# liuzuxin/FSRL

Hardware: NVIDIA H100
Metric: env-steps/sec (collect+update) SafetyCarCircle-v0 PPO-Lag (higher is better)
Workload: dtype f32

## Files before the change

fsrl_b200/csrc/mlp.cuh:

```cuda
#pragma once
#include "arena.cuh"
#include <cuda_pipeline.h>

namespace fsrl {

constexpr int MLP_TPB = 256;
constexpr int MLP_KC = 16;
constexpr int MLP_NST = 4;
constexpr int MLP_MAX_OUT = 16;
constexpr int MLP_MAX_IN = 64;

template <int H>
struct MlpTile {
    static_assert(H == 64 || H == 128 || H == 256 || H == 512, "hidden width must be 64/128/256/512");
    static constexpr int R = (4096 / H) < 16 ? 16 : (4096 / H);
    static constexpr int MT = R / 16;
    static constexpr int WN = H / 8;
    static constexpr int NT = WN / 8;
    static constexpr int LDA = H + 4;
    static constexpr int LDW = H + 8;
    static constexpr int PARTS = MLP_TPB / R;
    static constexpr int NST = (H >= 512) ? 2 : MLP_NST;
    __host__ __device__ static constexpr int in_pad(int in) { return ((in + 7) & ~7) + 4; }
    __host__ __device__ static constexpr int stage_floats() { return NST * MLP_KC * LDW; }
    __host__ __device__ static constexpr size_t smem_floats(int in, int out) {
        return (size_t)R * in_pad(in) + 2 * (size_t)R * LDA + stage_floats() + (size_t)H * out;
    }
    __host__ __device__ static constexpr size_t smem_bytes(int in, int out = MLP_MAX_OUT) {
        return sizeof(float) * smem_floats(in, out);
    }
};

__device__ __forceinline__ uint32_t round_tf32(float x) { return (__float_as_uint(x) + 0x1000u) & 0xffffe000u; }
__device__ __forceinline__ void split_tf32(float x, uint32_t& hi, uint32_t& lo) {
    hi = round_tf32(x);
    lo = round_tf32(x - __uint_as_float(hi));
}

__device__ __forceinline__ void mma_tf32(float (&c)[4], const uint32_t (&a)[4], const uint32_t (&b)[2]) {
    asm(
        "mma.sync.aligned.m16n8k8.row.col.f32.tf32.tf32.f32 {%0,%1,%2,%3}, {%4,%5,%6,%7}, {%8,%9}, {%0,%1,%2,%3};"
        : "+f"(c[0]), "+f"(c[1]), "+f"(c[2]), "+f"(c[3])
        : "r"(a[0]), "r"(a[1]), "r"(a[2]), "r"(a[3]), "r"(b[0]), "r"(b[1]));
}

template <int H>
__device__ __forceinline__ void stage_load(const float* mat, int K, float* wst, int chunk, int buf) {
    using TT = MlpTile<H>;
    float* dst = wst + (size_t)buf * MLP_KC * TT::LDW;
    constexpr int SEG = H / 4;
    for (int i = threadIdx.x; i < MLP_KC * SEG; i += MLP_TPB) {
        const int rr = i / SEG, sg = i % SEG;
        const int k = chunk * MLP_KC + rr;
        float* d = dst + (size_t)rr * TT::LDW + 4 * sg;
        if (k < K) __pipeline_memcpy_async(d, mat + (size_t)k * H + 4 * sg, 16);
        else *reinterpret_cast<float4*>(d) = make_float4(0.f, 0.f, 0.f, 0.f);
    }
    __pipeline_commit();
}

template <int H>
__device__ __forceinline__ void tc_gemm(float (&c)[MlpTile<H>::MT][MlpTile<H>::NT][4], const float* A,
                                        int lda, int K, const float* W, float* wst,
                                        bool stage0_in_flight) {
    using TT = MlpTile<H>;
    const int lane = threadIdx.x & 31, warp = threadIdx.x >> 5;
    const int g = lane >> 2, t = lane & 3;
    const int n0 = warp * TT::WN;
    const int Kp = (K + 7) & ~7;
    const int nch = (Kp + MLP_KC - 1) / MLP_KC;
    for (int p = stage0_in_flight ? 1 : 0; p < TT::NST - 1; ++p) {
        if (p < nch) stage_load<H>(W, K, wst, p, p);
        else __pipeline_commit();
    }
    for (int ch = 0; ch < nch; ++ch) {
        if (ch + TT::NST - 1 < nch) stage_load<H>(W, K, wst, ch + TT::NST - 1, (ch + TT::NST - 1) % TT::NST);
        else __pipeline_commit();
        __pipeline_wait_prior(TT::NST - 1);
        __syncthreads();
        const float* w = wst + (size_t)(ch % TT::NST) * MLP_KC * TT::LDW;
        const int kleft = Kp - ch * MLP_KC;
#pragma unroll
        for (int ks = 0; ks < MLP_KC; ks += 8) {
            if (ks < kleft) {
                const int k0 = ch * MLP_KC + ks;
                uint32_t bh[TT::NT][2], bl[TT::NT][2];
#pragma unroll
                for (int nt = 0; nt < TT::NT; ++nt) {
                    split_tf32(w[(size_t)(ks + t) * TT::LDW + n0 + 8 * nt + g], bh[nt][0], bl[nt][0]);
                    split_tf32(w[(size_t)(ks + t + 4) * TT::LDW + n0 + 8 * nt + g], bh[nt][1], bl[nt][1]);
                }
#pragma unroll
                for (int mt = 0; mt < TT::MT; ++mt) {
                    uint32_t ah[4], al[4];
                    const float* a = A + (size_t)(16 * mt + g) * lda + k0 + t;
                    split_tf32(a[0], ah[0], al[0]);
                    split_tf32(a[(size_t)8 * lda], ah[1], al[1]);
                    split_tf32(a[4], ah[2], al[2]);
                    split_tf32(a[(size_t)8 * lda + 4], ah[3], al[3]);
#pragma unroll
                    for (int nt = 0; nt < TT::NT; ++nt) mma_tf32(c[mt][nt], al, bh[nt]);
#pragma unroll
                    for (int nt = 0; nt < TT::NT; ++nt) mma_tf32(c[mt][nt], ah, bl[nt]);
#pragma unroll
                    for (int nt = 0; nt < TT::NT; ++nt) mma_tf32(c[mt][nt], ah, bh[nt]);
                }
            }
        }
        __syncthreads();
    }
}

template <int H, class F>
__device__ __forceinline__ void tc_foreach(float (&c)[MlpTile<H>::MT][MlpTile<H>::NT][4], F f) {
    using TT = MlpTile<H>;
    const int lane = threadIdx.x & 31, warp = threadIdx.x >> 5;
    const int g = lane >> 2, t = lane & 3;
#pragma unroll
    for (int mt = 0; mt < TT::MT; ++mt)
#pragma unroll
        for (int nt = 0; nt < TT::NT; ++nt) {
            const int col = warp * TT::WN + 8 * nt + 2 * t;
            f(16 * mt + g, col, c[mt][nt][0], c[mt][nt][1]);
            f(16 * mt + g + 8, col, c[mt][nt][2], c[mt][nt][3]);
        }
}

template <int H>
__device__ __forceinline__ void tc_init_bias(float (&c)[MlpTile<H>::MT][MlpTile<H>::NT][4], const float* bias) {
    using TT = MlpTile<H>;
    const int lane = threadIdx.x & 31, warp = threadIdx.x >> 5;
    const int t = lane & 3;
#pragma unroll
    for (int nt = 0; nt < TT::NT; ++nt) {
        const int col = warp * TT::WN + 8 * nt + 2 * t;
        const float b0 = bias ? __ldg(bias + col) : 0.f, b1 = bias ? __ldg(bias + col + 1) : 0.f;
#pragma unroll
        for (int mt = 0; mt < TT::MT; ++mt) { c[mt][nt][0] = b0; c[mt][nt][1] = b1; c[mt][nt][2] = b0; c[mt][nt][3] = b1; }
    }
}


constexpr int SLAB_NS = 64;
constexpr int SLAB_LDB = SLAB_NS + 8;
constexpr int SLAB_LDR = SLAB_NS + 4;

template <int H>
__host__ __device__ constexpr size_t slab_b_floats() { return (size_t)H * SLAB_LDB; }
template <int H>
__host__ __device__ constexpr size_t slab_red_floats() { return (size_t)8 * MlpTile<H>::R * SLAB_LDR; }
template <int H>
__host__ __device__ constexpr size_t slab_buf_floats() {
    return slab_b_floats<H>() > slab_red_floats<H>() ? slab_b_floats<H>() : slab_red_floats<H>();
}

template <int H>
__device__ __forceinline__ void slab_load(const float* W, int gld, int c0, float* bs) {
    constexpr int SEG = SLAB_NS / 4;
    for (int i = threadIdx.x; i < H * SEG; i += MLP_TPB) {
        const int k = i / SEG, sg = i % SEG;
        __pipeline_memcpy_async(bs + (size_t)k * SLAB_LDB + 4 * sg, W + (size_t)k * gld + c0 + 4 * sg, 16);
    }
    __pipeline_commit();
}

template <int H, class F>
__device__ __forceinline__ void slab_gemm(const float* A, int lda, const float* bs, float* red, F epi) {
    using TT = MlpTile<H>;
    constexpr int NTS = SLAB_NS / 8;
    constexpr int KW = H / 8;
    const int lane = threadIdx.x & 31, warp = threadIdx.x >> 5;
    const int g = lane >> 2, t = lane & 3;
    float c[TT::MT][NTS][4];
#pragma unroll
    for (int mt = 0; mt < TT::MT; ++mt)
#pragma unroll
        for (int nt = 0; nt < NTS; ++nt) { c[mt][nt][0] = c[mt][nt][1] = c[mt][nt][2] = c[mt][nt][3] = 0.f; }
#pragma unroll
    for (int ks = 0; ks < KW; ks += 8) {
        const int k0 = warp * KW + ks;
        uint32_t bh[NTS][2], bl[NTS][2];
#pragma unroll
        for (int nt = 0; nt < NTS; ++nt) {
            split_tf32(bs[(size_t)(k0 + t) * SLAB_LDB + 8 * nt + g], bh[nt][0], bl[nt][0]);
            split_tf32(bs[(size_t)(k0 + t + 4) * SLAB_LDB + 8 * nt + g], bh[nt][1], bl[nt][1]);
        }
#pragma unroll
        for (int mt = 0; mt < TT::MT; ++mt) {
            uint32_t ah[4], al[4];
            const float* a = A + (size_t)(16 * mt + g) * lda + k0 + t;
            split_tf32(a[0], ah[0], al[0]);
            split_tf32(a[(size_t)8 * lda], ah[1], al[1]);
            split_tf32(a[4], ah[2], al[2]);
            split_tf32(a[(size_t)8 * lda + 4], ah[3], al[3]);
#pragma unroll
            for (int nt = 0; nt < NTS; ++nt) mma_tf32(c[mt][nt], al, bh[nt]);
#pragma unroll
            for (int nt = 0; nt < NTS; ++nt) mma_tf32(c[mt][nt], ah, bl[nt]);
#pragma unroll
            for (int nt = 0; nt < NTS; ++nt) mma_tf32(c[mt][nt], ah, bh[nt]);
        }
    }
    __pipeline_wait_prior(0);
    __syncthreads();
    float* mine = red + (size_t)warp * TT::R * SLAB_LDR;
#pragma unroll
    for (int mt = 0; mt < TT::MT; ++mt)
#pragma unroll
        for (int nt = 0; nt < NTS; ++nt) {
            *reinterpret_cast<float2*>(mine + (size_t)(16 * mt + g) * SLAB_LDR + 8 * nt + 2 * t) = make_float2(c[mt][nt][0], c[mt][nt][1]);
            *reinterpret_cast<float2*>(mine + (size_t)(16 * mt + g + 8) * SLAB_LDR + 8 * nt + 2 * t) = make_float2(c[mt][nt][2], c[mt][nt][3]);
        }
    __syncthreads();
    for (int e = threadIdx.x; e < TT::R * (SLAB_NS / 4); e += MLP_TPB) {
        const int row = e / (SLAB_NS / 4), c4 = (e % (SLAB_NS / 4)) * 4;
        float4 s = make_float4(0.f, 0.f, 0.f, 0.f);
#pragma unroll
        for (int w = 0; w < 8; ++w) {
            const float4 v = *reinterpret_cast<const float4*>(red + ((size_t)w * TT::R + row) * SLAB_LDR + c4);
            s.x += v.x; s.y += v.y; s.z += v.z; s.w += v.w;
        }
        epi(row, c4, s);
    }
}

template <int H>
__device__ __forceinline__ void tc_gemm_direct(float (&c)[MlpTile<H>::MT][MlpTile<H>::NT][4], const float* A,
                                               int lda, int K, const float* W) {
    using TT = MlpTile<H>;
    const int lane = threadIdx.x & 31, warp = threadIdx.x >> 5;
    const int g = lane >> 2, t = lane & 3;
    const int n0 = warp * TT::WN;
    const int Kp = (K + 7) & ~7;
    for (int k0 = 0; k0 < Kp; k0 += 8) {
        uint32_t bh[TT::NT][2], bl[TT::NT][2];
#pragma unroll
        for (int nt = 0; nt < TT::NT; ++nt) {
            const float w0 = (k0 + t < K) ? __ldg(W + (size_t)(k0 + t) * H + n0 + 8 * nt + g) : 0.f;
            const float w1 = (k0 + t + 4 < K) ? __ldg(W + (size_t)(k0 + t + 4) * H + n0 + 8 * nt + g) : 0.f;
            split_tf32(w0, bh[nt][0], bl[nt][0]);
            split_tf32(w1, bh[nt][1], bl[nt][1]);
        }
#pragma unroll
        for (int mt = 0; mt < TT::MT; ++mt) {
            uint32_t ah[4], al[4];
            const float* a = A + (size_t)(16 * mt + g) * lda + k0 + t;
            split_tf32(a[0], ah[0], al[0]);
            split_tf32(a[(size_t)8 * lda], ah[1], al[1]);
            split_tf32(a[4], ah[2], al[2]);
            split_tf32(a[(size_t)8 * lda + 4], ah[3], al[3]);
#pragma unroll
            for (int nt = 0; nt < TT::NT; ++nt) mma_tf32(c[mt][nt], al, bh[nt]);
#pragma unroll
            for (int nt = 0; nt < TT::NT; ++nt) mma_tf32(c[mt][nt], ah, bl[nt]);
#pragma unroll
            for (int nt = 0; nt < TT::NT; ++nt) mma_tf32(c[mt][nt], ah, bh[nt]);
        }
    }
}

template <int H>
struct MlpSmem {
    float *x, *h1, *h2, *wst, *w3s;
    __device__ MlpSmem(float* base, int in, int out) {
        using TT = MlpTile<H>;
        x = base;
        h1 = x + (size_t)TT::R * TT::in_pad(in);
        h2 = h1 + (size_t)TT::R * TT::LDA;
        wst = h2 + (size_t)TT::R * TT::LDA;
        w3s = wst + TT::stage_floats();
        (void)out;
    }
    __device__ float* end(int out) const { return w3s + (size_t)H * out; }
};

template <int H>
__device__ __forceinline__ void mlp_hidden_forward(const Mlp3& m, const MlpSmem<H>& s) {
    using TT = MlpTile<H>;
    const int inp = TT::in_pad(m.in);
    for (int i = threadIdx.x; i < H * m.out; i += MLP_TPB) s.w3s[i] = __ldg(m.w3t + i);
    float c[TT::MT][TT::NT][4];
    tc_init_bias<H>(c, m.b1);
    tc_gemm<H>(c, s.x, inp, m.in, m.w1t, s.wst, false);
    stage_load<H>(m.w2t, H, s.wst, 0, 0);
    tc_foreach<H>(c, [&](int row, int col, float v0, float v1) {
        *reinterpret_cast<float2*>(s.h1 + (size_t)row * TT::LDA + col) = make_float2(fmaxf(v0, 0.f), fmaxf(v1, 0.f));
    });
    tc_init_bias<H>(c, m.b2);
    tc_gemm<H>(c, s.h1, TT::LDA, H, m.w2t, s.wst, true);
    tc_foreach<H>(c, [&](int row, int col, float v0, float v1) {
        *reinterpret_cast<float2*>(s.h2 + (size_t)row * TT::LDA + col) = make_float2(fmaxf(v0, 0.f), fmaxf(v1, 0.f));
    });
    __syncthreads();
}

template <int H>
__device__ __forceinline__ void mlp_head_forward(const Mlp3& m, const MlpSmem<H>& s, float* out) {
    using TT = MlpTile<H>;
    const int tid = threadIdx.x;
    const int r = tid / TT::PARTS, part = tid % TT::PARTS;
    const int no = m.out;
#pragma unroll
    for (int j = 0; j < MLP_MAX_OUT; ++j) out[j] = 0.f;
    for (int k = part; k < H; k += TT::PARTS) {
        const float x = s.h2[(size_t)r * TT::LDA + k];
        const float* w = s.w3s + (size_t)k * no;
#pragma unroll
        for (int j = 0; j < MLP_MAX_OUT; ++j)
            if (j < no) out[j] = fmaf(x, w[j], out[j]);
    }
#pragma unroll
    for (int j = 0; j < MLP_MAX_OUT; ++j) {
        if (j < no) {
            float v = out[j];
#pragma unroll
            for (int o = TT::PARTS / 2; o > 0; o >>= 1) v += __shfl_down_sync(0xffffffffu, v, o, TT::PARTS);
            out[j] = v + __ldg(m.b3 + j);
        }
    }
}

template <int H, class RowPtr>
__device__ __forceinline__ void mlp_stage_rows(const MlpSmem<H>& s, int in, RowPtr row_ptr) {
    using TT = MlpTile<H>;
    const int inp = TT::in_pad(in);
    for (int i = threadIdx.x; i < TT::R * inp; i += MLP_TPB) {
        const int r = i / inp, k = i % inp;
        const float* p = row_ptr(r);
        s.x[i] = (p != nullptr && k < in) ? p[k] : 0.f;
    }
}

}
```

fsrl_b200/csrc/mlpfwd.cu:

```cuda
#include "mlp.cuh"
#include "fsrl_b200.h"

namespace fsrl {

template <int H>
__global__ void __launch_bounds__(MLP_TPB)
mlp_forward_kernel(const Mlp3 m, const float* __restrict__ x, const int* __restrict__ idx,
                   long long n_rows, float* __restrict__ y) {
    using TT = MlpTile<H>;
    extern __shared__ __align__(16) float smem[];
    const int tid = threadIdx.x;
    const MlpSmem<H> sm(smem, m.in, m.out);
    const long long r0 = (long long)blockIdx.x * TT::R;
    mlp_stage_rows<H>(sm, m.in, [&](int r) -> const float* {
        const long long row = r0 + r;
        if (row >= n_rows) return nullptr;
        const long long src = idx ? (long long)idx[row] : row;
        return x + src * m.in;
    });
    __syncthreads();
    mlp_hidden_forward<H>(m, sm);
    float out[MLP_MAX_OUT];
    mlp_head_forward<H>(m, sm, out);
    const int r = tid / TT::PARTS, part = tid % TT::PARTS;
    const long long row = r0 + r;
    if (part == 0 && row < n_rows) {
#pragma unroll
        for (int j = 0; j < MLP_MAX_OUT; ++j)
            if (j < m.out) y[row * m.out + j] = out[j];
    }
}

}

using namespace fsrl;

extern "C" int fsrl_mlp_forward(const fsrl_mlp3_t* net, const float* x, const int* idx,
                                long long n_rows, float* y, void* stream) {
    FSRL_REQUIRE(n_rows >= 0, "fsrl_mlp_forward: n_rows < 0");
    if (n_rows == 0) return FSRL_OK;
    FSRL_REQUIRE(net && x && y, "fsrl_mlp_forward: null pointer");
    FSRL_REQUIRE(net->out >= 1 && net->out <= MLP_MAX_OUT, "fsrl_mlp_forward: out dim %d unsupported", net->out);
    if (n_rows == 0) return FSRL_OK;
    const Mlp3 m = *reinterpret_cast<const Mlp3*>(net);
    cudaStream_t s = static_cast<cudaStream_t>(stream);
#define GO(HH)                                                                                     \
    {                                                                                              \
        using TT = MlpTile<HH>;                                                                    \
        const size_t smem = TT::smem_bytes(m.in);                                                  \
        FSRL_CUDA(cudaFuncSetAttribute(mlp_forward_kernel<HH>, cudaFuncAttributeMaxDynamicSharedMemorySize, (int)smem)); \
        const long long grid = (n_rows + TT::R - 1) / TT::R;                                       \
        mlp_forward_kernel<HH><<<(unsigned)grid, MLP_TPB, smem, s>>>(m, x, idx, n_rows, y);        \
    }
    switch (m.H) {
        case 64: GO(64) break;
        case 128: GO(128) break;
        case 256: GO(256) break;
        case 512: GO(512) break;
        default: set_error("fsrl_mlp_forward: hidden width %d unsupported (64/128/256/512)", m.H); return FSRL_EINVAL;
    }
#undef GO
    FSRL_LAUNCH_CHECK();
    return FSRL_OK;
}
```

fsrl_b200/csrc/rollout.cu:

```cuda
#include "envs.cuh"
#include "mlp.cuh"
#include "fsrl_b200.h"

namespace fsrl {

static_assert(sizeof(fsrl_mlp3_t) == sizeof(Mlp3), "ABI struct mismatch");
static_assert(FSRL_BOUND_CLIP == 1 && FSRL_BOUND_TANH == 2, "map_action() codes");

template <int KIND>
__device__ __forceinline__ void collect_step_tail(const fsrl_rollout_t& a, int e, const float* obs,
                                                  const float* act, float logp) {
    using E_ = Env<KIND>;
    constexpr int D = E_::D, A = E_::A, S = E_::S;
    fsrl_collect_stats_t* st = a.stats;
    float aenv[A];
#pragma unroll
    for (int j = 0; j < A; ++j)
        aenv[j] = map_action(act[j], a.action_bound, a.action_scaling, a.act_low[j], a.act_high[j]);
    float s[S];
#pragma unroll
    for (int i = 0; i < S; ++i) s[i] = a.env_state[(size_t)i * a.E + e];
    float rew, cost;
    bool term;
    const uint32_t ep = a.ep_idx[e] - 1u;
    E_::step(s, aenv, a.seed_env, (uint32_t)e, ep, rew, cost, term);
    const int t_new = a.env_t[e] + 1;
    const bool trunc = (t_new >= a.max_steps) && !term;
    const bool done = term || trunc;
    float on[D];
    E_::observe(s, on, a.seed_env, (uint32_t)e, ep);

    if (a.b_obs) {
        const int ptr = a.b_ptr[e];
        const size_t p = (size_t)e * a.cap + ptr;
#pragma unroll
        for (int k = 0; k < D; ++k) {
            a.b_obs[p * D + k] = obs[k];
            a.b_obs_next[p * D + k] = on[k];
        }
#pragma unroll
        for (int j = 0; j < A; ++j) a.b_act[p * A + j] = act[j];
        a.b_rew[p] = rew; a.b_cost[p] = cost; a.b_logp[p] = logp;
        a.b_term[p] = term ? 1 : 0; a.b_trunc[p] = trunc ? 1 : 0;
        a.b_ptr[e] = (ptr + 1 == a.cap) ? 0 : ptr + 1;
        const int len = a.b_len[e];
        if (len < a.cap) a.b_len[e] = len + 1;
    }
    atomicAdd(&st->step_count, 1ull);
    if (cost != 0.f) atomicAdd(&st->total_cost, (double)cost);
    const double er = a.ep_rew[e] + (double)rew;
    const int el = a.ep_len[e] + 1;
    a.ep_rew[e] = er; a.ep_len[e] = el;
    a.env_t[e] = t_new;

    if (done) {
        if (a.inline_done) {
            atomicAdd(&st->sum_ep_rew, er);
            atomicAdd(&st->sum_ep_len, (unsigned long long)el);
            atomicAdd(term ? &st->term_count : &st->trunc_count, 1);
            a.active[e] = 0;
            a.ep_rew[e] = 0.0; a.ep_len[e] = 0;
            const int c = atomicAdd(&st->episode_count, 1) + 1;
            if (c >= st->n_episode) st->finished_next = 1;
        } else {
            a.done_now[e] = term ? 1 : 2;
        }
    }
#pragma unroll
    for (int i = 0; i < S; ++i) a.env_state[(size_t)i * a.E + e] = s[i];
#pragma unroll
    for (int k = 0; k < D; ++k) a.obs_cur[(size_t)e * D + k] = on[k];
}

template <int KIND, int H>
__global__ void __launch_bounds__(MLP_TPB)
rollout_step_kernel(const fsrl_rollout_t a) {
    using E_ = Env<KIND>;
    using TT = MlpTile<H>;
    constexpr int D = E_::D, A = E_::A;
    extern __shared__ __align__(16) float smem[];
    fsrl_collect_stats_t* st = a.stats;
    if (st->finished) return;

    const int tid = threadIdx.x;
    const int e0 = blockIdx.x * TT::R;
    const Mlp3& actor = *reinterpret_cast<const Mlp3*>(&a.actor);
    const MlpSmem<H> sm(smem, D, actor.out);
    constexpr int INP = TT::in_pad(D);
    float* xtile = sm.x;

    __shared__ int s_any;
    if (tid == 0) s_any = 0;
    __syncthreads();
    if (tid < TT::R) {
        const int e = e0 + tid;
        if (e < a.E && a.active[e]) s_any = 1;
    }
    __syncthreads();
    if (!s_any) return;

    mlp_stage_rows<H>(sm, D, [&](int r) -> const float* {
        const int e = e0 + r;
        return e < a.E ? a.obs_cur + (size_t)e * D : nullptr;
    });
    __syncthreads();

    float out[MLP_MAX_OUT];
    if (a.mode != FSRL_MODE_RANDOM) {
        mlp_hidden_forward<H>(actor, sm);
        mlp_head_forward<H>(actor, sm, out);
    }

    const int r = tid / TT::PARTS, part = tid % TT::PARTS;
    const int e = e0 + r;
    if (part != 0 || e >= a.E || !a.active[e]) return;

    float act[A], mu[A], sig[A];
    float logp = 0.f;
    const uint32_t ctr = a.act_ctr[e];
    float eps[(A + 3) / 4 * 4];
    if (a.mode == FSRL_MODE_TRAIN || a.mode == FSRL_MODE_RANDOM) {
#pragma unroll
        for (int c = 0; c < (A + 3) / 4; ++c) {
            uint32_t rr[4];
            Philox::gen((uint32_t)e, ctr, (uint32_t)c, 0u, a.seed_act, KEY_ACT, rr);
            if (a.mode == FSRL_MODE_RANDOM) {
#pragma unroll
                for (int j = 0; j < 4; ++j) eps[4 * c + j] = usym(rr[j]);
            } else {
                gauss_pair(rr[0], rr[1], eps[4 * c], eps[4 * c + 1]);
                gauss_pair(rr[2], rr[3], eps[4 * c + 2], eps[4 * c + 3]);
            }
        }
        a.act_ctr[e] = ctr + 1u;
    }
#pragma unroll
    for (int j = 0; j < A; ++j) {
        if (a.mode == FSRL_MODE_RANDOM) {
            float v = eps[j];
            if (a.action_bound == FSRL_BOUND_TANH) v = 0.5f * (log1pf(v) - log1pf(-v));
            act[j] = v; mu[j] = 0.f; sig[j] = 1.f;
            continue;
        }
        if (a.head == FSRL_HEAD_GAUSS_INDEP) {
            mu[j] = a.bounded ? a.max_action * tanhf(out[j]) : out[j];
            sig[j] = expf(__ldg(a.log_sigma + j));
        } else if (a.head == FSRL_HEAD_GAUSS_COND || a.head == FSRL_HEAD_GAUSS_COND_RAW) {
            mu[j] = a.bounded ? a.max_action * tanhf(out[j]) : out[j];
            sig[j] = expf(fminf(fmaxf(out[A + j], a.sigma_min), a.sigma_max));
        } else {
            mu[j] = a.max_action * tanhf(out[j]);
            sig[j] = 0.f;
        }
        if (a.mode == FSRL_MODE_EVAL || a.head == FSRL_HEAD_DETERMINISTIC) act[j] = mu[j];
        else act[j] = fmaf(sig[j], eps[j], mu[j]);
    }
    if (a.head == FSRL_HEAD_GAUSS_COND && a.mode != FSRL_MODE_RANDOM) {
        float lp = 0.f;
#pragma unroll
        for (int j = 0; j < A; ++j) {
            const float z = (a.mode == FSRL_MODE_EVAL) ? 0.f : eps[j];
            lp += -0.5f * z * z - logf(sig[j]) - LOG_SQRT_2PI;
            const float sq = tanhf(act[j]);
            lp -= logf(1.0f - sq * sq + a.tanh_eps);
            act[j] = sq;
        }
        logp = lp;
    } else if ((a.head == FSRL_HEAD_GAUSS_INDEP || a.head == FSRL_HEAD_GAUSS_COND_RAW) && a.mode != FSRL_MODE_RANDOM) {
        float lp = 0.f;
#pragma unroll
        for (int j = 0; j < A; ++j) {
            const float z = (act[j] - mu[j]) / sig[j];
            lp += -0.5f * z * z - logf(sig[j]) - LOG_SQRT_2PI;
        }
        logp = lp;
    }
    if (a.head == FSRL_HEAD_DETERMINISTIC && a.mode == FSRL_MODE_TRAIN && a.expl_sigma > 0.f) {
#pragma unroll
        for (int j = 0; j < A; ++j) act[j] = fmaf(a.expl_sigma, eps[j], act[j]);
    }
    collect_step_tail<KIND>(a, e, xtile + r * INP, act, logp);
}

template <int KIND>
__global__ void __launch_bounds__(128) rollout_act_step_kernel(const fsrl_rollout_t a, const float* __restrict__ act_in) {
    constexpr int D = Env<KIND>::D, A = Env<KIND>::A;
    if (a.stats->finished) return;
    const int e = blockIdx.x * blockDim.x + threadIdx.x;
    if (e >= a.E || !a.active[e]) return;
    float act[A];
#pragma unroll
    for (int j = 0; j < A; ++j) act[j] = act_in[(size_t)e * A + j];
    collect_step_tail<KIND>(a, e, a.obs_cur + (size_t)e * D, act, 0.f);
}

template <int KIND>
__global__ void __launch_bounds__(1024) rollout_resolve_kernel(const fsrl_rollout_t a) {
    using E_ = Env<KIND>;
    constexpr int D = E_::D, S = E_::S;
    fsrl_collect_stats_t* st = a.stats;
    __shared__ int s_scan[1024];
    __shared__ int s_base, s_total, s_surplus;
    const int tid = threadIdx.x;
    if (st->finished) return;
    if (st->finished_next) {
        if (tid == 0) st->finished = 1;
        return;
    }
    if (a.inline_done) return;
    int local = 0;
    for (int e = tid; e < a.E; e += 1024) local += (a.active[e] && a.done_now[e]) ? 1 : 0;
    s_scan[tid] = local;
    __syncthreads();
    for (int o = 512; o > 0; o >>= 1) {
        if (tid < o) s_scan[tid] += s_scan[tid + o];
        __syncthreads();
    }
    if (tid == 0) {
        s_total = s_scan[0];
        const int epc = st->episode_count + s_total;
        int surplus = st->n_ready - (st->n_episode - epc);
        if (surplus < 0) surplus = 0;
        if (surplus > s_total) surplus = s_total;
        s_surplus = surplus;
        s_base = 0;
    }
    __syncthreads();
    const int total = s_total;
    if (total == 0) return;
    const int surplus = s_surplus;
    for (int c0 = 0; c0 < a.E; c0 += 1024) {
        const int e = c0 + tid;
        const int flag = (e < a.E && a.active[e] && a.done_now[e]) ? 1 : 0;
        s_scan[tid] = flag;
        __syncthreads();
        for (int o = 1; o < 1024; o <<= 1) {
            int v = (tid >= o) ? s_scan[tid - o] : 0;
            __syncthreads();
            s_scan[tid] += v;
            __syncthreads();
        }
        const int rank = s_base + s_scan[tid] - flag;
        if (flag) {
            const bool term = a.done_now[e] == 1;
            atomicAdd(&st->sum_ep_rew, a.ep_rew[e]);
            atomicAdd(&st->sum_ep_len, (unsigned long long)a.ep_len[e]);
            atomicAdd(term ? &st->term_count : &st->trunc_count, 1);
            a.ep_rew[e] = 0.0; a.ep_len[e] = 0; a.done_now[e] = 0;
            if (rank < surplus) {
                a.active[e] = 0;
            } else {
                float s[S], o[D];
                const uint32_t ep = a.ep_idx[e];
                E_::reset(s, a.seed_env, (uint32_t)e, ep);
                a.ep_idx[e] = ep + 1u;
                a.env_t[e] = 0;
                E_::observe(s, o, a.seed_env, (uint32_t)e, ep);
                for (int i = 0; i < S; ++i) a.env_state[(size_t)i * a.E + e] = s[i];
                for (int k = 0; k < D; ++k) a.obs_cur[(size_t)e * D + k] = o[k];
            }
        }
        __syncthreads();
        if (tid == 1023) s_base += s_scan[1023];
        __syncthreads();
    }
    if (tid == 0) {
        st->episode_count += total;
        st->n_ready -= surplus;
        if (st->episode_count >= st->n_episode) st->finished = 1;
    }
}

template <int KIND>
__device__ __forceinline__ void env_reset_one(const fsrl_rollout_t& a, int e, float* o) {
    using E_ = Env<KIND>;
    constexpr int D = E_::D, S = E_::S;
    float s[S];
    const uint32_t ep = a.ep_idx[e];
    E_::reset(s, a.seed_env, (uint32_t)e, ep);
    a.ep_idx[e] = ep + 1u;
    a.env_t[e] = 0;
    a.ep_rew[e] = 0.0; a.ep_len[e] = 0; a.done_now[e] = 0;
    E_::observe(s, o, a.seed_env, (uint32_t)e, ep);
    for (int i = 0; i < S; ++i) a.env_state[(size_t)i * a.E + e] = s[i];
    for (int k = 0; k < D; ++k) a.obs_cur[(size_t)e * D + k] = o[k];
}

template <int KIND>
__global__ void env_reset_all_kernel(const fsrl_rollout_t a) {
    const int e = blockIdx.x * blockDim.x + threadIdx.x;
    if (e >= a.E) return;
    float o[Env<KIND>::D];
    env_reset_one<KIND>(a, e, o);
}

constexpr int ENV_IDS_CHUNK = 512;
struct EnvIds {
    int n, i0, all, pad;
    int e[ENV_IDS_CHUNK];
};

__device__ __forceinline__ int env_of_row(const EnvIds& ids, int k) { return ids.all ? ids.i0 + k : ids.e[k]; }

template <int KIND>
__global__ void __launch_bounds__(128) env_reset_ids_kernel(const fsrl_rollout_t a, const __grid_constant__ EnvIds ids,
                                                            float* __restrict__ obs) {
    constexpr int D = Env<KIND>::D;
    const int k = blockIdx.x * blockDim.x + threadIdx.x;
    if (k >= ids.n) return;
    float o[D];
    env_reset_one<KIND>(a, env_of_row(ids, k), o);
    if (obs) {
        const size_t i = (size_t)(ids.i0 + k);
#pragma unroll
        for (int c = 0; c < D; ++c) obs[i * D + c] = o[c];
    }
}

template <int KIND>
__global__ void __launch_bounds__(128) env_step_ids_kernel(const fsrl_rollout_t a, const __grid_constant__ EnvIds ids,
                                                           const float* __restrict__ act, float* __restrict__ obs_next,
                                                           float* __restrict__ rew_out, float* __restrict__ cost_out,
                                                           uint8_t* __restrict__ term_out, uint8_t* __restrict__ trunc_out) {
    using E_ = Env<KIND>;
    constexpr int D = E_::D, A = E_::A, S = E_::S;
    const int k = blockIdx.x * blockDim.x + threadIdx.x;
    if (k >= ids.n) return;
    const size_t i = (size_t)(ids.i0 + k);
    const int e = env_of_row(ids, k);
    float aenv[A];
#pragma unroll
    for (int j = 0; j < A; ++j) aenv[j] = act[i * A + j];
    float s[S];
#pragma unroll
    for (int c = 0; c < S; ++c) s[c] = a.env_state[(size_t)c * a.E + e];
    float rew, cost;
    bool term;
    const uint32_t ep = a.ep_idx[e] - 1u;
    E_::step(s, aenv, a.seed_env, (uint32_t)e, ep, rew, cost, term);
    const int t_new = a.env_t[e] + 1;
    const bool trunc = (t_new >= a.max_steps) && !term;
    float on[D];
    E_::observe(s, on, a.seed_env, (uint32_t)e, ep);
    a.ep_rew[e] += (double)rew;
    a.ep_len[e] += 1;
    a.env_t[e] = t_new;
#pragma unroll
    for (int c = 0; c < S; ++c) a.env_state[(size_t)c * a.E + e] = s[c];
#pragma unroll
    for (int c = 0; c < D; ++c) {
        a.obs_cur[(size_t)e * D + c] = on[c];
        obs_next[i * D + c] = on[c];
    }
    rew_out[i] = rew; cost_out[i] = cost;
    term_out[i] = term ? 1 : 0; trunc_out[i] = trunc ? 1 : 0;
}

__global__ void collect_begin_kernel(const fsrl_rollout_t a, int n_episode) {
    fsrl_collect_stats_t* st = a.stats;
    const int e = blockIdx.x * blockDim.x + threadIdx.x;
    const int ready = n_episode < a.E ? n_episode : a.E;
    if (e < a.E) { a.active[e] = e < ready ? 1 : 0; a.done_now[e] = 0; a.ep_rew[e] = 0.0; a.ep_len[e] = 0; }
    if (e == 0) {
        st->step_count = 0; st->total_cost = 0.0; st->sum_ep_rew = 0.0; st->sum_ep_len = 0;
        st->episode_count = 0; st->n_episode = n_episode; st->n_ready = ready;
        st->term_count = 0; st->trunc_count = 0; st->finished = 0; st->finished_next = 0;
    }
}

template <int KIND>
static int launch_step_h(const fsrl_rollout_t& a, cudaStream_t s) {
    const int H = a.actor.H;
#define GO(HH)                                                                                   \
    {                                                                                            \
        using TT = MlpTile<HH>;                                                                  \
        const size_t smem = TT::smem_bytes(Env<KIND>::D);                                        \
        static bool attr_done = false;                                                           \
        if (!attr_done) {                                                                        \
            FSRL_CUDA(cudaFuncSetAttribute(rollout_step_kernel<KIND, HH>,                        \
                                           cudaFuncAttributeMaxDynamicSharedMemorySize, (int)smem)); \
            attr_done = true;                                                                    \
        }                                                                                        \
        const int grid = (a.E + TT::R - 1) / TT::R;                                              \
        rollout_step_kernel<KIND, HH><<<grid, MLP_TPB, smem, s>>>(a);                            \
    }
    switch (H) {
        case 64: GO(64) break;
        case 128: GO(128) break;
        case 256: GO(256) break;
        case 512: GO(512) break;
        default: set_error("rollout: hidden width %d unsupported (64/128/256/512)", H); return FSRL_EINVAL;
    }
#undef GO
    FSRL_LAUNCH_CHECK();
    rollout_resolve_kernel<KIND><<<1, 1024, 0, s>>>(a);
    FSRL_LAUNCH_CHECK();
    return FSRL_OK;
}

template <int KIND>
static int launch_act_step(const fsrl_rollout_t& a, const float* act, cudaStream_t s) {
    rollout_act_step_kernel<KIND><<<(a.E + 127) / 128, 128, 0, s>>>(a, act);
    FSRL_LAUNCH_CHECK();
    rollout_resolve_kernel<KIND><<<1, 1024, 0, s>>>(a);
    FSRL_LAUNCH_CHECK();
    return FSRL_OK;
}

template <typename F>
static int for_id_chunks(const int32_t* ids, int n, F&& launch) {
    EnvIds c;
    c.pad = 0;
    c.all = ids == nullptr;
    const int step = ids ? ENV_IDS_CHUNK : n;
    for (int i0 = 0; i0 < n; i0 += step) {
        c.i0 = i0;
        c.n = n - i0 < step ? n - i0 : step;
        if (ids)
            for (int k = 0; k < c.n; ++k) c.e[k] = ids[i0 + k];
        int rc = launch(c);
        if (rc) return rc;
    }
    return FSRL_OK;
}

template <int KIND>
static int launch_env_step(const fsrl_rollout_t& a, const float* act, const int32_t* ids, int n, float* obs_next,
                           float* rew, float* cost, uint8_t* term, uint8_t* trunc, cudaStream_t s) {
    return for_id_chunks(ids, n, [&](const EnvIds& c) {
        env_step_ids_kernel<KIND><<<(c.n + 127) / 128, 128, 0, s>>>(a, c, act, obs_next, rew, cost, term, trunc);
        FSRL_LAUNCH_CHECK();
        return FSRL_OK;
    });
}

template <int KIND>
static int launch_env_reset_ids(const fsrl_rollout_t& a, const int32_t* ids, int n, float* obs, cudaStream_t s) {
    return for_id_chunks(ids, n, [&](const EnvIds& c) {
        env_reset_ids_kernel<KIND><<<(c.n + 127) / 128, 128, 0, s>>>(a, c, obs);
        FSRL_LAUNCH_CHECK();
        return FSRL_OK;
    });
}

}

using namespace fsrl;

static int check_env_state(const fsrl_rollout_t* a) {
    FSRL_REQUIRE(a != nullptr, "rollout: null descriptor");
    FSRL_REQUIRE(env_kind_known(a->kind), "rollout: unknown env kind %d", a->kind);
    FSRL_REQUIRE(a->E > 0, "rollout: E must be positive");
    FSRL_REQUIRE(a->env_state && a->obs_cur && a->env_t && a->ep_idx && a->act_ctr && a->active &&
                 a->ep_rew && a->ep_len && a->done_now && a->stats, "rollout: null state pointer");
    return FSRL_OK;
}

static int check_rollout(const fsrl_rollout_t* a) {
    int rc = check_env_state(a);
    if (rc) return rc;
    const EnvDims d = env_dims(a->kind);
    FSRL_REQUIRE(a->actor.in == d.D || a->mode == FSRL_MODE_RANDOM, "rollout: actor input dim %d != obs dim %d", a->actor.in, d.D);
    return FSRL_OK;
}

static int check_ids(const char* fn, const fsrl_rollout_t* a, const int32_t* ids, int n) {
    FSRL_REQUIRE(n >= 1 && n <= a->E, "%s: n = %d outside [1, E = %d]", fn, n, a->E);
    FSRL_REQUIRE(ids != nullptr || n == a->E, "%s: without ids, n must be E = %d (got %d)", fn, a->E, n);
    if (ids)
        for (int i = 0; i < n; ++i)
            FSRL_REQUIRE(ids[i] >= 0 && ids[i] < a->E, "%s: ids[%d] = %d outside [0, E = %d)", fn, i, ids[i], a->E);
    return FSRL_OK;
}

#define DISPATCH_KIND(kind, CALL)                                                    \
    switch (kind) {                                                                  \
        case ENV_CAR_CIRCLE: { constexpr int K = ENV_CAR_CIRCLE; CALL; } break;      \
        case ENV_CAR_RUN: { constexpr int K = ENV_CAR_RUN; CALL; } break;            \
        case ENV_BALL_CIRCLE: { constexpr int K = ENV_BALL_CIRCLE; CALL; } break;    \
        case ENV_BALL_RUN: { constexpr int K = ENV_BALL_RUN; CALL; } break;          \
        case ENV_ANT_CIRCLE: { constexpr int K = ENV_ANT_CIRCLE; CALL; } break;      \
        case ENV_POINT_GOAL: { constexpr int K = ENV_POINT_GOAL; CALL; } break;      \
        case ENV_ANT_RUN: { constexpr int K = ENV_ANT_RUN; CALL; } break;            \
        case ENV_DRONE_CIRCLE: { constexpr int K = ENV_DRONE_CIRCLE; CALL; } break;  \
        case ENV_DRONE_RUN: { constexpr int K = ENV_DRONE_RUN; CALL; } break;        \
        case ENV_POINT_CIRCLE1: { constexpr int K = ENV_POINT_CIRCLE1; CALL; } break;\
        case ENV_POINT_CIRCLE2: { constexpr int K = ENV_POINT_CIRCLE2; CALL; } break;\
        case ENV_CAR_CIRCLE1: { constexpr int K = ENV_CAR_CIRCLE1; CALL; } break;    \
        case ENV_CAR_CIRCLE2: { constexpr int K = ENV_CAR_CIRCLE2; CALL; } break;    \
        case ENV_POINT_GOAL2: { constexpr int K = ENV_POINT_GOAL2; CALL; } break;    \
        case ENV_CAR_GOAL1: { constexpr int K = ENV_CAR_GOAL1; CALL; } break;        \
        case ENV_CAR_GOAL2: { constexpr int K = ENV_CAR_GOAL2; CALL; } break;        \
        default: set_error("unknown env kind %d", kind); return FSRL_EINVAL;         \
    }

extern "C" int fsrl_env_dims(int kind, int* D, int* A, int* S, int* T) {
    FSRL_REQUIRE(env_kind_known(kind), "fsrl_env_dims: unknown env kind %d", kind);
    const EnvDims d = env_dims(kind);
    if (D) *D = d.D; if (A) *A = d.A; if (S) *S = d.S; if (T) *T = d.T;
    return FSRL_OK;
}

extern "C" int fsrl_env_reset_all(const fsrl_rollout_t* a, void* stream) {
    int rc = check_rollout(a);
    if (rc) return rc;
    cudaStream_t s = static_cast<cudaStream_t>(stream);
    DISPATCH_KIND(a->kind, (env_reset_all_kernel<K><<<(a->E + 127) / 128, 128, 0, s>>>(*a)));
    FSRL_LAUNCH_CHECK();
    return FSRL_OK;
}

extern "C" int fsrl_collect_begin(const fsrl_rollout_t* a, int n_episode, void* stream) {
    int rc = check_env_state(a);
    if (rc) return rc;
    FSRL_REQUIRE(n_episode > 0, "n_episode must be positive");
    cudaStream_t s = static_cast<cudaStream_t>(stream);
    collect_begin_kernel<<<(a->E + 127) / 128, 128, 0, s>>>(*a, n_episode);
    FSRL_LAUNCH_CHECK();
    return FSRL_OK;
}

extern "C" int fsrl_rollout_steps(const fsrl_rollout_t* a, int n_steps, void* stream) {
    int rc = check_rollout(a);
    if (rc) return rc;
    FSRL_REQUIRE(n_steps >= 0, "fsrl_rollout_steps: n_steps < 0");
    FSRL_REQUIRE(a->mode == FSRL_MODE_RANDOM || (a->actor.w1t && a->actor.w2t && a->actor.w3t),
                 "rollout: null actor weights");
    FSRL_REQUIRE(a->actor.out <= MLP_MAX_OUT, "rollout: actor out dim %d > %d", a->actor.out, MLP_MAX_OUT);
    cudaStream_t s = static_cast<cudaStream_t>(stream);
    for (int i = 0; i < n_steps; ++i) {
        DISPATCH_KIND(a->kind, { int r2 = launch_step_h<K>(*a, s); if (r2) return r2; });
    }
    return FSRL_OK;
}

extern "C" int fsrl_rollout_steps_act(const fsrl_rollout_t* a, const float* act, void* stream) {
    int rc = check_env_state(a);
    if (rc) return rc;
    FSRL_REQUIRE(act != nullptr, "fsrl_rollout_steps_act: null action array");
    cudaStream_t s = static_cast<cudaStream_t>(stream);
    DISPATCH_KIND(a->kind, rc = launch_act_step<K>(*a, act, s));
    return rc;
}

extern "C" int fsrl_env_step(const fsrl_rollout_t* a, const float* act, const int32_t* ids, int n, float* obs_next,
                             float* rew, float* cost, uint8_t* term, uint8_t* trunc, void* stream) {
    int rc = check_env_state(a);
    if (rc) return rc;
    rc = check_ids("fsrl_env_step", a, ids, n);
    if (rc) return rc;
    FSRL_REQUIRE(act && obs_next && rew && cost && term && trunc, "fsrl_env_step: null action or output array");
    cudaStream_t s = static_cast<cudaStream_t>(stream);
    DISPATCH_KIND(a->kind, rc = launch_env_step<K>(*a, act, ids, n, obs_next, rew, cost, term, trunc, s));
    return rc;
}

extern "C" int fsrl_env_reset_ids(const fsrl_rollout_t* a, const int32_t* ids, int n, float* obs, void* stream) {
    int rc = check_env_state(a);
    if (rc) return rc;
    rc = check_ids("fsrl_env_reset_ids", a, ids, n);
    if (rc) return rc;
    cudaStream_t s = static_cast<cudaStream_t>(stream);
    DISPATCH_KIND(a->kind, rc = launch_env_reset_ids<K>(*a, ids, n, obs, s));
    return rc;
}
```

Measured before the change: 2.549 million.

## Fuse multi-step rollout into one persistent kernel and add row-tiled MLP forward

```diff
diff --git a/fsrl_b200/csrc/mlp.cuh b/fsrl_b200/csrc/mlp.cuh
--- a/fsrl_b200/csrc/mlp.cuh
+++ b/fsrl_b200/csrc/mlp.cuh
@@ -59,8 +59,8 @@
     __pipeline_commit();
 }
 
-template <int H>
-__device__ __forceinline__ void tc_gemm(float (&c)[MlpTile<H>::MT][MlpTile<H>::NT][4], const float* A,
+template <int H, int MT = MlpTile<H>::MT>
+__device__ __forceinline__ void tc_gemm(float (&c)[MT][MlpTile<H>::NT][4], const float* A,
                                         int lda, int K, const float* W, float* wst,
                                         bool stage0_in_flight) {
     using TT = MlpTile<H>;
@@ -91,7 +91,7 @@
                     split_tf32(w[(size_t)(ks + t + 4) * TT::LDW + n0 + 8 * nt + g], bh[nt][1], bl[nt][1]);
                 }
 #pragma unroll
-                for (int mt = 0; mt < TT::MT; ++mt) {
+                for (int mt = 0; mt < MT; ++mt) {
                     uint32_t ah[4], al[4];
                     const float* a = A + (size_t)(16 * mt + g) * lda + k0 + t;
                     split_tf32(a[0], ah[0], al[0]);
@@ -111,13 +111,13 @@
     }
 }
 
-template <int H, class F>
-__device__ __forceinline__ void tc_foreach(float (&c)[MlpTile<H>::MT][MlpTile<H>::NT][4], F f) {
+template <int H, int MT = MlpTile<H>::MT, class F>
+__device__ __forceinline__ void tc_foreach(float (&c)[MT][MlpTile<H>::NT][4], F f) {
     using TT = MlpTile<H>;
     const int lane = threadIdx.x & 31, warp = threadIdx.x >> 5;
     const int g = lane >> 2, t = lane & 3;
 #pragma unroll
-    for (int mt = 0; mt < TT::MT; ++mt)
+    for (int mt = 0; mt < MT; ++mt)
 #pragma unroll
         for (int nt = 0; nt < TT::NT; ++nt) {
             const int col = warp * TT::WN + 8 * nt + 2 * t;
@@ -126,8 +126,8 @@
         }
 }
 
-template <int H>
-__device__ __forceinline__ void tc_init_bias(float (&c)[MlpTile<H>::MT][MlpTile<H>::NT][4], const float* bias) {
+template <int H, int MT = MlpTile<H>::MT>
+__device__ __forceinline__ void tc_init_bias(float (&c)[MT][MlpTile<H>::NT][4], const float* bias) {
     using TT = MlpTile<H>;
     const int lane = threadIdx.x & 31, warp = threadIdx.x >> 5;
     const int t = lane & 3;
@@ -136,7 +136,7 @@
         const int col = warp * TT::WN + 8 * nt + 2 * t;
         const float b0 = bias ? __ldg(bias + col) : 0.f, b1 = bias ? __ldg(bias + col + 1) : 0.f;
 #pragma unroll
-        for (int mt = 0; mt < TT::MT; ++mt) { c[mt][nt][0] = b0; c[mt][nt][1] = b1; c[mt][nt][2] = b0; c[mt][nt][3] = b1; }
+        for (int mt = 0; mt < MT; ++mt) { c[mt][nt][0] = b0; c[mt][nt][1] = b1; c[mt][nt][2] = b0; c[mt][nt][3] = b1; }
     }
 }
 
@@ -295,7 +295,7 @@
 }
 
 template <int H>
-__device__ __forceinline__ void mlp_head_forward(const Mlp3& m, const MlpSmem<H>& s, float* out) {
+__device__ __forceinline__ void mlp_head_forward(const Mlp3& m, const float* h2, const float* w3s, float* out) {
     using TT = MlpTile<H>;
     const int tid = threadIdx.x;
     const int r = tid / TT::PARTS, part = tid % TT::PARTS;
@@ -303,8 +303,8 @@
 #pragma unroll
     for (int j = 0; j < MLP_MAX_OUT; ++j) out[j] = 0.f;
     for (int k = part; k < H; k += TT::PARTS) {
-        const float x = s.h2[(size_t)r * TT::LDA + k];
-        const float* w = s.w3s + (size_t)k * no;
+        const float x = h2[(size_t)r * TT::LDA + k];
+        const float* w = w3s + (size_t)k * no;
 #pragma unroll
         for (int j = 0; j < MLP_MAX_OUT; ++j)
             if (j < no) out[j] = fmaf(x, w[j], out[j]);
@@ -318,6 +318,11 @@
             out[j] = v + __ldg(m.b3 + j);
         }
     }
+}
+
+template <int H>
+__device__ __forceinline__ void mlp_head_forward(const Mlp3& m, const MlpSmem<H>& s, float* out) {
+    mlp_head_forward<H>(m, s.h2, s.w3s, out);
 }
 
 template <int H, class RowPtr>
diff --git a/fsrl_b200/csrc/mlpfwd.cu b/fsrl_b200/csrc/mlpfwd.cu
--- a/fsrl_b200/csrc/mlpfwd.cu
+++ b/fsrl_b200/csrc/mlpfwd.cu
@@ -1,5 +1,6 @@
 #include "mlp.cuh"
 #include "fsrl_b200.h"
+#include <cstdlib>
 
 namespace fsrl {
 
@@ -31,6 +32,102 @@
     }
 }
 
+constexpr int FWD_ROWS = 64;
+
+template <int H>
+__host__ __device__ constexpr size_t fwd_rows_smem_bytes(int in, int out) {
+    using TT = MlpTile<H>;
+    return sizeof(float) * ((size_t)FWD_ROWS * TT::in_pad(in) + (size_t)FWD_ROWS * TT::LDA + TT::stage_floats() +
+                            (size_t)H * out);
+}
+
+template <int H>
+__global__ void __launch_bounds__(MLP_TPB)
+mlp_forward_rows_kernel(const Mlp3 m, const float* __restrict__ x, const int* __restrict__ idx,
+                        long long n_rows, float* __restrict__ y) {
+    using TT = MlpTile<H>;
+    constexpr int MT = FWD_ROWS / 16;
+    static_assert(FWD_ROWS % TT::R == 0, "the head runs in passes of MlpTile<H>::R rows");
+    extern __shared__ __align__(16) float smem[];
+    const int tid = threadIdx.x;
+    const int inp = TT::in_pad(m.in);
+    float* xs = smem;
+    float* hs = xs + (size_t)FWD_ROWS * inp;
+    float* wst = hs + (size_t)FWD_ROWS * TT::LDA;
+    float* w3s = wst + TT::stage_floats();
+    for (int i = tid; i < H * m.out; i += MLP_TPB) w3s[i] = __ldg(m.w3t + i);
+    const long long n_tiles = (n_rows + FWD_ROWS - 1) / FWD_ROWS;
+    for (long long tile = blockIdx.x; tile < n_tiles; tile += gridDim.x) {
+        const long long r0 = tile * FWD_ROWS;
+        for (int i = tid; i < FWD_ROWS * inp; i += MLP_TPB) {
+            const int r = i / inp, k = i % inp;
+            const long long row = r0 + r;
+            float v = 0.f;
+            if (row < n_rows && k < m.in) v = x[(idx ? (long long)idx[row] : row) * m.in + k];
+            xs[i] = v;
+        }
+        float c[MT][TT::NT][4];
+        tc_init_bias<H, MT>(c, m.b1);
+        tc_gemm<H, MT>(c, xs, inp, m.in, m.w1t, wst, false);
+        stage_load<H>(m.w2t, H, wst, 0, 0);
+        tc_foreach<H, MT>(c, [&](int row, int col, float v0, float v1) {
+            *reinterpret_cast<float2*>(hs + (size_t)row * TT::LDA + col) = make_float2(fmaxf(v0, 0.f), fmaxf(v1, 0.f));
+        });
+        tc_init_bias<H, MT>(c, m.b2);
+        tc_gemm<H, MT>(c, hs, TT::LDA, H, m.w2t, wst, true);
+        tc_foreach<H, MT>(c, [&](int row, int col, float v0, float v1) {
+            *reinterpret_cast<float2*>(hs + (size_t)row * TT::LDA + col) = make_float2(fmaxf(v0, 0.f), fmaxf(v1, 0.f));
+        });
+        __syncthreads();
+        const int r = tid / TT::PARTS, part = tid % TT::PARTS;
+#pragma unroll 1
+        for (int p = 0; p < FWD_ROWS / TT::R; ++p) {
+            float out[MLP_MAX_OUT];
+            mlp_head_forward<H>(m, hs + (size_t)p * TT::R * TT::LDA, w3s, out);
+            const long long row = r0 + p * TT::R + r;
+            if (part == 0 && row < n_rows) {
+#pragma unroll
+                for (int j = 0; j < MLP_MAX_OUT; ++j)
+                    if (j < m.out) y[row * m.out + j] = out[j];
+            }
+        }
+    }
+}
+
+template <int H>
+static int rows_grid(size_t smem, long long n_tiles, long long* grid) {
+    static size_t cached_smem[64] = {0};
+    static int cached_per_sm[64] = {0};
+    int dev = 0;
+    FSRL_CUDA(cudaGetDevice(&dev));
+    FSRL_REQUIRE(dev >= 0 && dev < 64, "fsrl_mlp_forward: device %d", dev);
+    if (smem != cached_smem[dev]) {
+        int optin = 0, per_sm = 0;
+        FSRL_CUDA(cudaDeviceGetAttribute(&optin, cudaDevAttrMaxSharedMemoryPerBlockOptin, dev));
+        if (smem <= (size_t)optin) {
+            FSRL_CUDA(cudaFuncSetAttribute(mlp_forward_rows_kernel<H>, cudaFuncAttributeMaxDynamicSharedMemorySize, (int)smem));
+            FSRL_CUDA(cudaOccupancyMaxActiveBlocksPerMultiprocessor(&per_sm, mlp_forward_rows_kernel<H>, MLP_TPB, smem));
+        }
+        cached_per_sm[dev] = per_sm;
+        cached_smem[dev] = smem;
+    }
+    const long long cap = (long long)sm_count() * cached_per_sm[dev];
+    *grid = n_tiles < cap ? n_tiles : cap;
+    return FSRL_OK;
+}
+
+template <int H>
+static int launch_forward_rows(const Mlp3& m, const float* x, const int* idx, long long n_rows, float* y,
+                               cudaStream_t s, bool* launched) {
+    const size_t smem = fwd_rows_smem_bytes<H>(m.in, m.out);
+    long long grid = 0;
+    const int rc = rows_grid<H>(smem, (n_rows + FWD_ROWS - 1) / FWD_ROWS, &grid);
+    if (rc) return rc;
+    *launched = grid > 0;
+    if (*launched) mlp_forward_rows_kernel<H><<<(unsigned)grid, MLP_TPB, smem, s>>>(m, x, idx, n_rows, y);
+    return FSRL_OK;
+}
+
 }
 
 using namespace fsrl;
@@ -44,6 +141,8 @@
     if (n_rows == 0) return FSRL_OK;
     const Mlp3 m = *reinterpret_cast<const Mlp3*>(net);
     cudaStream_t s = static_cast<cudaStream_t>(stream);
+    const char* tiled = getenv("FSRL_MLPFWD_TILED");
+    const bool rows = !(tiled && atoi(tiled) != 0);
 #define GO(HH)                                                                                     \
     {                                                                                              \
         using TT = MlpTile<HH>;                                                                    \
@@ -54,8 +153,16 @@
     }
     switch (m.H) {
         case 64: GO(64) break;
-        case 128: GO(128) break;
-        case 256: GO(256) break;
+        case 128: {
+            bool done = false;
+            if (rows) { int rc = launch_forward_rows<128>(m, x, idx, n_rows, y, s, &done); if (rc) return rc; }
+            if (!done) GO(128)
+        } break;
+        case 256: {
+            bool done = false;
+            if (rows) { int rc = launch_forward_rows<256>(m, x, idx, n_rows, y, s, &done); if (rc) return rc; }
+            if (!done) GO(256)
+        } break;
         case 512: GO(512) break;
         default: set_error("fsrl_mlp_forward: hidden width %d unsupported (64/128/256/512)", m.H); return FSRL_EINVAL;
     }
diff --git a/fsrl_b200/csrc/rollout.cu b/fsrl_b200/csrc/rollout.cu
--- a/fsrl_b200/csrc/rollout.cu
+++ b/fsrl_b200/csrc/rollout.cu
@@ -1,6 +1,7 @@
 #include "envs.cuh"
 #include "mlp.cuh"
 #include "fsrl_b200.h"
+#include <cstdlib>
 
 namespace fsrl {
 
@@ -72,49 +73,9 @@
     for (int k = 0; k < D; ++k) a.obs_cur[(size_t)e * D + k] = on[k];
 }
 
-template <int KIND, int H>
-__global__ void __launch_bounds__(MLP_TPB)
-rollout_step_kernel(const fsrl_rollout_t a) {
-    using E_ = Env<KIND>;
-    using TT = MlpTile<H>;
-    constexpr int D = E_::D, A = E_::A;
-    extern __shared__ __align__(16) float smem[];
-    fsrl_collect_stats_t* st = a.stats;
-    if (st->finished) return;
-
-    const int tid = threadIdx.x;
-    const int e0 = blockIdx.x * TT::R;
-    const Mlp3& actor = *reinterpret_cast<const Mlp3*>(&a.actor);
-    const MlpSmem<H> sm(smem, D, actor.out);
-    constexpr int INP = TT::in_pad(D);
-    float* xtile = sm.x;
-
-    __shared__ int s_any;
-    if (tid == 0) s_any = 0;
-    __syncthreads();
-    if (tid < TT::R) {
-        const int e = e0 + tid;
-        if (e < a.E && a.active[e]) s_any = 1;
-    }
-    __syncthreads();
-    if (!s_any) return;
-
-    mlp_stage_rows<H>(sm, D, [&](int r) -> const float* {
-        const int e = e0 + r;
-        return e < a.E ? a.obs_cur + (size_t)e * D : nullptr;
-    });
-    __syncthreads();
-
-    float out[MLP_MAX_OUT];
-    if (a.mode != FSRL_MODE_RANDOM) {
-        mlp_hidden_forward<H>(actor, sm);
-        mlp_head_forward<H>(actor, sm, out);
-    }
-
-    const int r = tid / TT::PARTS, part = tid % TT::PARTS;
-    const int e = e0 + r;
-    if (part != 0 || e >= a.E || !a.active[e]) return;
-
+template <int KIND>
+__device__ __forceinline__ void fused_step_env(const fsrl_rollout_t& a, int e, const float* out, const float* obs) {
+    constexpr int A = Env<KIND>::A;
     float act[A], mu[A], sig[A];
     float logp = 0.f;
     const uint32_t ctr = a.act_ctr[e];
@@ -179,7 +140,54 @@
 #pragma unroll
         for (int j = 0; j < A; ++j) act[j] = fmaf(a.expl_sigma, eps[j], act[j]);
     }
-    collect_step_tail<KIND>(a, e, xtile + r * INP, act, logp);
+    collect_step_tail<KIND>(a, e, obs, act, logp);
+}
+
+template <int KIND, int H>
+__global__ void __launch_bounds__(MLP_TPB, 1)
+rollout_step_kernel(const fsrl_rollout_t a, int n_steps) {
+    using E_ = Env<KIND>;
+    using TT = MlpTile<H>;
+    constexpr int D = E_::D;
+    extern __shared__ __align__(16) float smem[];
+    fsrl_collect_stats_t* st = a.stats;
+    if (st->finished) return;
+
+    const int tid = threadIdx.x;
+    const int e0 = blockIdx.x * TT::R;
+    const Mlp3& actor = *reinterpret_cast<const Mlp3*>(&a.actor);
+    const MlpSmem<H> sm(smem, D, actor.out);
+    constexpr int INP = TT::in_pad(D);
+    float* xtile = sm.x;
+    const int r = tid / TT::PARTS, part = tid % TT::PARTS;
+    const int e = e0 + r;
+
+    __shared__ int s_any;
+    for (int step = 0; step < n_steps; ++step) {
+        if (tid == 0) s_any = 0;
+        __syncthreads();
+        if (tid < TT::R) {
+            const int et = e0 + tid;
+            if (et < a.E && a.active[et]) s_any = 1;
+        }
+        __syncthreads();
+        if (!s_any) return;
+
+        mlp_stage_rows<H>(sm, D, [&](int rr) -> const float* {
+            const int et = e0 + rr;
+            return et < a.E ? a.obs_cur + (size_t)et * D : nullptr;
+        });
+        __syncthreads();
+
+        float out[MLP_MAX_OUT];
+        if (a.mode != FSRL_MODE_RANDOM) {
+            mlp_hidden_forward<H>(actor, sm);
+            mlp_head_forward<H>(actor, sm, out);
+        }
+
+        if (part == 0 && e < a.E && a.active[e]) fused_step_env<KIND>(a, e, out, xtile + r * INP);
+        __syncthreads();
+    }
 }
 
 template <int KIND>
@@ -369,7 +377,7 @@
 }
 
 template <int KIND>
-static int launch_step_h(const fsrl_rollout_t& a, cudaStream_t s) {
+static int launch_steps_h(const fsrl_rollout_t& a, int n_steps, bool one_launch, cudaStream_t s) {
     const int H = a.actor.H;
 #define GO(HH)                                                                                   \
     {                                                                                            \
@@ -382,7 +390,19 @@
             attr_done = true;                                                                    \
         }                                                                                        \
         const int grid = (a.E + TT::R - 1) / TT::R;                                              \
-        rollout_step_kernel<KIND, HH><<<grid, MLP_TPB, smem, s>>>(a);                            \
+        if (one_launch) {                                                                        \
+            rollout_step_kernel<KIND, HH><<<grid, MLP_TPB, smem, s>>>(a, n_steps);               \
+            FSRL_LAUNCH_CHECK();                                                                 \
+            rollout_resolve_kernel<KIND><<<1, 1024, 0, s>>>(a);                                  \
+            FSRL_LAUNCH_CHECK();                                                                 \
+        } else {                                                                                 \
+            for (int i = 0; i < n_steps; ++i) {                                                  \
+                rollout_step_kernel<KIND, HH><<<grid, MLP_TPB, smem, s>>>(a, 1);                 \
+                FSRL_LAUNCH_CHECK();                                                             \
+                rollout_resolve_kernel<KIND><<<1, 1024, 0, s>>>(a);                              \
+                FSRL_LAUNCH_CHECK();                                                             \
+            }                                                                                    \
+        }                                                                                        \
     }
     switch (H) {
         case 64: GO(64) break;
@@ -392,9 +412,6 @@
         default: set_error("rollout: hidden width %d unsupported (64/128/256/512)", H); return FSRL_EINVAL;
     }
 #undef GO
-    FSRL_LAUNCH_CHECK();
-    rollout_resolve_kernel<KIND><<<1, 1024, 0, s>>>(a);
-    FSRL_LAUNCH_CHECK();
     return FSRL_OK;
 }
 
@@ -527,11 +544,12 @@
     FSRL_REQUIRE(a->mode == FSRL_MODE_RANDOM || (a->actor.w1t && a->actor.w2t && a->actor.w3t),
                  "rollout: null actor weights");
     FSRL_REQUIRE(a->actor.out <= MLP_MAX_OUT, "rollout: actor out dim %d > %d", a->actor.out, MLP_MAX_OUT);
+    if (n_steps == 0) return FSRL_OK;
     cudaStream_t s = static_cast<cudaStream_t>(stream);
-    for (int i = 0; i < n_steps; ++i) {
-        DISPATCH_KIND(a->kind, { int r2 = launch_step_h<K>(*a, s); if (r2) return r2; });
-    }
-    return FSRL_OK;
+    const char* per_step = getenv("FSRL_ROLLOUT_PER_STEP");
+    const bool one_launch = a->inline_done && !(per_step && atoi(per_step) != 0);
+    DISPATCH_KIND(a->kind, rc = launch_steps_h<K>(*a, n_steps, one_launch, s));
+    return rc;
 }
 
 extern "C" int fsrl_rollout_steps_act(const fsrl_rollout_t* a, const float* act, void* stream) {
```

New measurement: 2.639 million (median of 6 runs). 1.04x the previous value.
